# orangeai-research/Generative-Multimodal-Recommendation

Hardware: AMD Instinct MI355X
Metric: train users/sec + full-rank eval users/sec, DiffMM Amazon-baby, 1/2/4/8 MI355X (higher is better)
Workload: dtype fp32; 1 GPU; DiffMM baby-shaped synthetic: 19445 users x 7050 items, 121517 train interactions; step = one DiffMMTrainer epoch (diffusion train + graph rebuild + BPR/contrastive); global_batch=2048, eval_batch=4096, parallelism=dp1

## Files before the change

### generative-multimodal-recommendation_amd/csrc/gemm.hip

```cpp
#include <stdlib.h>

#include <type_traits>

#include "gemm_impl.h"

namespace {
using namespace gmr_gemm;

template <int BM, int BN, int WGM, int WGN, bool AKC, bool BKC, bool VEC, int MF>
__global__ void __launch_bounds__(64 * WGM * WGN) gemm_kernel(int64_t M, int64_t N, int64_t K,
                                                             const float* __restrict__ A, int64_t lda,
                                                             const float* __restrict__ B, int64_t ldb,
                                                             float* __restrict__ C, int64_t ldc, Epi epi, int tiles_n,
                                                             int64_t k_per_split, float* __restrict__ ws) {
  constexpr int NT = 64 * WGM * WGN;
  constexpr int WTM = BM / WGM, WTN = BN / WGN;
  constexpr int TM = WTM / MF, TN = WTN / MF;
  using AccT = typename std::conditional<MF == 32, floatx16, floatx4>::type;
  constexpr int NE = MF == 32 ? 16 : 4;
  using SA = Stage<BM, AKC, VEC, NT>;
  using SB = Stage<BN, BKC, VEC, NT>;
  __shared__ __attribute__((aligned(16))) float smem[2 * (SA::WORDS + SB::WORDS)];
  constexpr int STAGE_WORDS = SA::WORDS + SB::WORDS;

// ... 428 lines not shown
                 int64_t K, const float* A, int64_t lda, const float* B, int64_t ldb, float* C, int64_t ldc,
                 const Epi& epi, int tiles_n, int64_t kps, float* ws, int* counters, bool x6p) {
  if (mf == 6)
    return launch_mf<BM, BN, WGM, WGN, 6>(ta, tb, vec, false, grid, st, M, N, K, A, lda, B, ldb, C, ldc, epi, tiles_n, kps, ws,
                                   counters, x6p);
  else if (mf == 16)
    return launch_mf<BM, BN, WGM, WGN, 16>(ta, tb, vec, false, grid, st, M, N, K, A, lda, B, ldb, C, ldc, epi, tiles_n, kps,
                                    ws, counters, x6p);
  else
    return launch_mf<BM, BN, WGM, WGN, 32>(ta, tb, vec, glds, grid, st, M, N, K, A, lda, B, ldb, C, ldc, epi, tiles_n, kps,
                                    ws, counters, x6p);
}

struct Plan {
  int tile, bm, bn, splits, mf;
  bool glds;
  int64_t tm, tn, kps;
  int xpose;
  bool x6p;
};

int default_mfma() {
  static int mf = [] {
    const char* e = getenv("GMR_GEMM_MFMA");
    return (e && atoi(e) == 16) ? 16 : 32;
  }();
  return mf;
}

bool default_x6() {
  static bool x = [] {
    const char* e = getenv("GMR_GEMM_X6");
    return !(e && atoi(e) == 0);
  }();
  return x;
}

bool default_x6_64() {
  static bool x = [] {
    const char* e = getenv("GMR_GEMM_X6_64");
    return !(e && atoi(e) == 0);
  }();
  return x;
}

bool default_glds() {
  static bool g = [] {
    const char* e = getenv("GMR_GEMM_GLDS");
    return !(e && atoi(e) == 0);
  }();
  return g;
}

int auto_splits(int64_t tm, int64_t tn, int bm, int64_t K) {
  const bool skinny = bm == 64 && (tm == 1 || tn == 1);
  const int64_t min_k = skinny ? 192 : 512;
  const int max_s = skinny ? 64 : 16;
  int s = 1;
  while (tm * tn * s < 512 && K / (s * 2) >= min_k && s < max_s) s *= 2;
  if (bm == 128) {
    const int64_t slots = 512;
    auto waves = [&](int q) { return (double)(tm * tn * q) / (double)slots; };
    auto fill = [&](int q) {
      const int64_t w = tm * tn * q;
      return (double)w / (double)(((w + slots - 1) / slots) * slots);
    };
    while ((waves(s) < 8.0 || fill(s) < 0.9) && K / (s * 2) >= min_k && s < max_s) s *= 2;
  }
  return s;
}

Plan make_plan_core(int ta, int tb, int64_t M, int64_t N, int64_t K, int tile, int split_k, bool allow_x6) {
  int mf = default_mfma();
  if (tile & GMR_GEMM_MFMA16) mf = 16;
  if (tile & GMR_GEMM_MFMA32) mf = 32;
  bool glds = default_glds();
  if (tile & GMR_GEMM_GLDS) glds = true;
  if (tile & GMR_GEMM_REGSTAGE) glds = false;
  const bool x6 = allow_x6 && ((tile & GMR_GEMM_X6) || default_x6()) &&
                  !(tile & (GMR_GEMM_F32 | GMR_GEMM_MFMA16 | GMR_GEMM_MFMA32 | GMR_GEMM_GLDS | GMR_GEMM_REGSTAGE));
  const bool x6_64 = x6 && ((tile & GMR_GEMM_X6) || default_x6_64());
  const bool x6_pipe1 = tile & GMR_GEMM_X6_PIPE1;
  tile &= ~(GMR_GEMM_MFMA16 | GMR_GEMM_MFMA32 | GMR_GEMM_GLDS | GMR_GEMM_REGSTAGE | GMR_GEMM_X6 | GMR_GEMM_F32 |
            GMR_GEMM_X6_PIPE1);
  if (tile == 0) {
    const bool tnm = ta && !tb;
    auto fill = [](int64_t tiles, int64_t slots) { return (double)tiles / (double)(((tiles + slots - 1) / slots) * slots); };
    const bool wide256 = M >= 2048 && N >= 4096 && K >= 256 && K <= 1024 &&
                         fill(((M + 255) / 256) * ((N + 255) / 256), 256) >=
                             0.92 * fill(((M + 127) / 128) * ((N + 127) / 128), 512);
    auto score = [&](int t) {
      const int64_t tm = (M + t - 1) / t, tn = (N + t - 1) / t;
      const int s = auto_splits(tm, tn, t, K);
      double pen = 1.0;
      for (int q = s; q > 1; q >>= 1) pen *= 0.95;
      return fill(tm * tn * s, t == 256 ? 256 : 512) * pen * (t == 256 ? 1.03 : 1.0);
    };
    if (!tnm && M >= 2048 && N >= 1000 && K >= 4096)
      tile = (tb || !glds) && score(256) >= score(128) ? 256 : 128;
    else if (!tnm && wide256) tile = 256;
    else if (!tnm && M * N >= (int64_t)8 << 20 && K >= 512) tile = 128;
    else if (!tnm && M * N >= (int64_t)1 << 20 && K >= 4096) tile = 128;
    else if (!ta && !tb && N <= 64 && M >= 4096 && K >= 2048) tile = 12864;
    else tile = 64;
  }
  if (x6 && tile == 64 && M * N >= ((int64_t)4 << 20) && K >= 256) tile = 128;
  if (x6 && (tile != 64 || x6_64) && tile != 12864 && !ta && tb) {
    mf = 6;
    if (tile == 256) tile = ((M + 127) / 128) * ((N + 127) / 128) >= 768 ? 128 : 256128;
  }
  Plan p;
  p.mf = mf;
  p.glds = glds && mf == 32;
  p.tile = tile;
  p.bm = tile == 256128 ? 256 : tile == 128256 || tile == 12864 ? 128 : tile;
  p.bn = tile == 256128 ? 128 : tile == 128256 ? 256 : tile == 12864 ? 64 : tile;
  p.tm = (M + p.bm - 1) / p.bm;
  p.tn = (N + p.bn - 1) / p.bn;
  int splits = split_k;
  if (splits <= 0 && mf == 6) {
    static const int64_t min_slab_env = [] {
      const char* e = getenv("GMR_X6_MIN_SLAB");
      const int v = e ? atoi(e) : 0;
      return (int64_t)(v >= 64 ? v : 0);
    }();
    const int64_t min_slab = min_slab_env ? min_slab_env : p.bm == 64 ? (x6_ring() && K <= 1024 ? K : 256) : 512;
    const int64_t slots = p.bm == 64 ? 768 : p.bm * p.bn == 128 * 128 ? 512 : 256;
    splits = 1;
    while (p.tm * p.tn * splits * 5 < slots * 4 && K / (splits * 2) >= min_slab && splits < 16) splits *= 2;
  }
  if (splits <= 0) splits = auto_splits(p.tm, p.tn, p.bm, K);
  int64_t kps = (K + splits - 1) / splits;
  kps = (kps + BK - 1) / BK * BK;
  p.splits = (int)((K + kps - 1) / kps);
  p.kps = kps;
  p.xpose = 0;
  p.x6p = mf == 6 && x6_pipe1;
  return p;
}

Plan make_plan(int ta, int tb, int64_t M, int64_t N, int64_t K, int tile, int split_k) {
  if (ta || !tb) {
    Plan q = make_plan_core(0, 1, M, N, K, tile, split_k, true);
    if (q.mf == 6 && q.bm != 64) {
      q.xpose = (ta ? 1 : 0) | (tb ? 0 : 2);
      return q;
    }
    return make_plan_core(ta, tb, M, N, K, tile, split_k, false);
  }
  return make_plan_core(ta, tb, M, N, K, tile, split_k, true);
}

struct WsLayout {
  int64_t slabs, at, bt, total, kp;
};
WsLayout ws_layout(const Plan& p, int64_t M, int64_t N, int64_t K) {
  auto r4 = [](int64_t v) { return (v + 3) / 4 * 4; };
  WsLayout w;
  w.kp = r4(K);
  const bool uses = p.splits > 1 || p.xpose;
  w.slabs = GMR_GEMM_COUNTER_WORDS;
  w.at = uses ? r4(GMR_GEMM_COUNTER_WORDS + (p.splits > 1 ? (int64_t)p.splits * M * N : 0)) : 0;
  w.bt = w.at + ((p.xpose & 1) ? r4(M * w.kp) : 0);
  w.total = w.bt + ((p.xpose & 2) ? r4(N * w.kp) : 0);
  return w;
}

}

extern "C" int32_t gmr_gemm_kernel_kind(int32_t trans_a, int32_t trans_b, int64_t M, int64_t N, int64_t K,
                                        int32_t tile, int32_t split_k, int32_t aligned) {
  if (M <= 0 || N <= 0 || K <= 0) return 0;
  const Plan p = make_plan(trans_a, trans_b, M, N, K, tile, split_k);
  if (p.mf == 6 && !aligned && p.xpose != 3)
    return make_plan_core(trans_a, trans_b, M, N, K, tile, split_k, false).mf;
  return p.mf;
}

extern "C" int64_t gmr_gemm_workspace_floats(int32_t trans_a, int32_t trans_b, int64_t M, int64_t N, int64_t K,
                                             int32_t tile, int32_t split_k) {
  if (M <= 0 || N <= 0 || K <= 0) return 0;
  const Plan p = make_plan(trans_a, trans_b, M, N, K, tile, split_k);
  int64_t need = ws_layout(p, M, N, K).total;
  if (p.mf == 6) {
    const Plan q = make_plan_core(trans_a, trans_b, M, N, K, tile, split_k, false);
    need = std::max(need, ws_layout(q, M, N, K).total);
  }
  return need;
}

extern "C" int gmr_gemm_f32(int32_t trans_a, int32_t trans_b, int64_t M, int64_t N, int64_t K, float alpha,
                            const float* A, int64_t lda, const float* B, int64_t ldb, float beta, float* C,
                            int64_t ldc, int32_t epilogue, const float* bias, const int32_t* bias_row, int64_t ld_bias,
                            const float* aux, int64_t ld_aux, const float* rowvec1, const float* rowvec2, float slope,
                            int32_t tile, int32_t split_k, float* workspace, int64_t workspace_floats, void* stream) {
  GMR_ARG(A && B && C, "null operand");
  GMR_ARG(M > 0 && N > 0 && K > 0, "empty GEMM");
  GMR_ARG(lda >= (trans_a ? M : K) && ldb >= (trans_b ? K : N) && ldc >= N, "leading dimension too small");
  GMR_ARG(epilogue >= GMR_EPI_NONE && epilogue <= GMR_EPI_SCALE_BIAS, "bad epilogue");
  GMR_ARG(epilogue != GMR_EPI_LEAKY_NORM ||
              (N == 64 && aux && rowvec1 && ld_aux >= 64 && ld_aux % 4 == 0 && ldc % 4 == 0 &&
               (((uintptr_t)aux | (uintptr_t)C) & 15) == 0),
          "GMR_EPI_LEAKY_NORM: N = 64, 16-byte aligned C and aux (the normalised rows), rowvec1 (the norms)");
  GMR_ARG(!(epilogue == GMR_EPI_POSTERIOR || epilogue == GMR_EPI_DTANH || epilogue == GMR_EPI_ROWSCALE_AUX ||
            epilogue == GMR_EPI_DRELU) || aux,
          "epilogue needs aux");
  GMR_ARG(epilogue != GMR_EPI_ROWSCALE_AUX || rowvec1, "epilogue needs rowvec1");
  {
    const int t = tile & ~(GMR_GEMM_MFMA16 | GMR_GEMM_MFMA32 | GMR_GEMM_GLDS | GMR_GEMM_REGSTAGE | GMR_GEMM_X6 |
                           GMR_GEMM_F32 | GMR_GEMM_X6_PIPE1);
    GMR_ARG(t == 0 || t == 64 || t == 128 || t == 256 || t == 256128 || t == 128256 || t == 12864,
            "tile must be 0 (auto), 64, 128, 256, 256128, 128256 or 12864 (| GMR_GEMM_MFMA16 / GMR_GEMM_MFMA32)");
  }
  Epi e;
  e.kind = epilogue;
  e.alpha = alpha;
  e.beta = beta;
  e.slope = slope;
  e.bias = bias;
  e.bias_row = bias_row;
  e.ld_bias = ld_bias;
  e.aux = aux;
  e.ld_aux = ld_aux;
  e.rv1 = rowvec1;
  e.rv2 = rowvec2;
  const bool a16 = ((uintptr_t)A % 16 == 0) && lda % 4 == 0, b16 = ((uintptr_t)B % 16 == 0) && ldb % 4 == 0;
  bool vec = a16 && b16;
  Plan pl = make_plan(trans_a, trans_b, M, N, K, tile, split_k);
  if (pl.mf == 6 && !(((pl.xpose & 1) || a16) && ((pl.xpose & 2) || b16)))
    pl = make_plan_core(trans_a, trans_b, M, N, K, tile, split_k, false);
  if ((pl.xpose & 2) && x6_inplace()) pl.xpose &= ~2;
  if (pl.xpose == 1 && !trans_b && x6_inplace() == 2) pl.xpose = 0;
  const WsLayout wl = ws_layout(pl, M, N, K);
  if (pl.xpose) {
    GMR_ARG(workspace && workspace_floats >= wl.total, "needs workspace of gmr_gemm_workspace_floats(...) floats");
    GMR_ARG(((uintptr_t)workspace & 15) == 0, "workspace must be 16-byte aligned");
    if (pl.xpose & 1) {
      x6_transpose(A, lda, K, M, workspace + wl.at, wl.kp, (hipStream_t)stream);
      GMR_LAUNCHED();
      A = workspace + wl.at;
      lda = wl.kp;
    }
    if (pl.xpose & 2) {
      x6_transpose(B, ldb, K, N, workspace + wl.bt, wl.kp, (hipStream_t)stream);
      GMR_LAUNCHED();
      B = workspace + wl.bt;
      ldb = wl.kp;
    }
    if (pl.xpose & 1) trans_a = 0;
    if (pl.xpose & 2) trans_b = 1;
    vec = (pl.xpose & 1 ? true : a16) && (pl.xpose & 2 ? true : b16);
  }
  tile = pl.tile;
  const int64_t tm = pl.tm, tn = pl.tn, kps = pl.kps;
  const int splits = pl.splits;
  GMR_ARG(tm * tn < (1ll << 31), "too many tiles");
  float* ws = nullptr;
  int* counters = nullptr;
  if (splits > 1) {
    GMR_ARG(workspace && workspace_floats >= GMR_GEMM_COUNTER_WORDS + (int64_t)splits * M * N,
            "split-K needs workspace of gmr_gemm_workspace_floats(...) floats");
    ws = workspace + GMR_GEMM_COUNTER_WORDS;
    if (pl.glds && vec && tm * tn <= GMR_GEMM_COUNTER_WORDS && inkernel_fixup() && epilogue != GMR_EPI_LEAKY_NORM)
      counters = reinterpret_cast<int*>(workspace);
  }
  GMR_ARG(epilogue != GMR_EPI_LEAKY_NORM || splits > 1, "GMR_EPI_LEAKY_NORM needs a split-K plan");
  hipStream_t st = (hipStream_t)stream;
  dim3 grid((unsigned)(tm * tn), 1, (unsigned)splits);
  const int tnp = (int)tn | (tile_group(tn) << 20);
  int lrc = 0;
  switch (tile) {
    case 256:
      lrc = launch_tile<256, 256, 4, 4>(pl.mf, pl.glds, trans_a, trans_b, vec, grid, st, M, N, K, A, lda, B, ldb, C, ldc, e, tnp, kps, ws, counters, pl.x6p);
      break;
    case 256128:
      lrc = launch_tile<256, 128, 4, 2>(pl.mf, pl.glds, trans_a, trans_b, vec, grid, st, M, N, K, A, lda, B, ldb, C, ldc, e, tnp, kps, ws, counters, pl.x6p);
      break;
    case 128256:
      lrc = launch_tile<128, 256, 2, 4>(pl.mf, pl.glds, trans_a, trans_b, vec, grid, st, M, N, K, A, lda, B, ldb, C, ldc, e, tnp, kps, ws, counters, pl.x6p);
      break;
    case 12864:
      lrc = launch_tile<128, 64, 2, 2>(pl.mf, pl.glds, trans_a, trans_b, vec, grid, st, M, N, K, A, lda, B, ldb, C, ldc, e, tnp, kps, ws, counters, pl.x6p);
      break;
    case 128:
      lrc = launch_tile<128, 128, 2, 2>(pl.mf, pl.glds, trans_a, trans_b, vec, grid, st, M, N, K, A, lda, B, ldb, C, ldc, e, tnp, kps, ws, counters, pl.x6p);
      break;
    default:
      lrc = launch_tile<64, 64, 2, 2>(pl.mf, pl.glds, trans_a, trans_b, vec, grid, st, M, N, K, A, lda, B, ldb, C, ldc, e, tnp, kps, ws, counters, pl.x6p);
  }
  GMR_ARG(lrc == 0, "no split-bf16 kernel for this tile and operand layout");
  GMR_LAUNCHED();
  if (ws && !counters && epilogue == GMR_EPI_LEAKY_NORM) {
    hipLaunchKernelGGL(splitk_reduce_leaky_norm_kernel, dim3(gmr::grid_for(M * 16, 256)), dim3(256), 0, st, M, splits,
                       ws, C, ldc, e, const_cast<float*>(aux), ld_aux, const_cast<float*>(rowvec1));
    GMR_LAUNCHED();
  } else if (ws && !counters) {
    hipLaunchKernelGGL(splitk_reduce_kernel, dim3(gmr::grid_for(M * N, 256)), dim3(256), 0, st, M, N, splits, ws, C,
                       ldc, e);
    GMR_LAUNCHED();
  }
  return GMR_OK;
}
```

### generative-multimodal-recommendation_amd/csrc/gemm_x6.hip

```cpp
#include <stdlib.h>

#include <type_traits>

#include "gemm_impl.h"
#include "x6_split.h"

namespace {
using namespace gmr_gemm;

typedef __bf16 bf16x8 __attribute__((ext_vector_type(8)));
typedef __bf16 bf16x4 __attribute__((ext_vector_type(4)));

__device__ __forceinline__ int x6_swz(int r) { return (r >> 2) & 3; }

__device__ __forceinline__ void split3(float x, __bf16& h, __bf16& m, __bf16& l) {
  h = (__bf16)__builtin_amdgcn_fmed3f(x, -0x1.fep127f, 0x1.fep127f);
  const float r1 = x - (float)h;
  m = (__bf16)r1;
  l = (__bf16)(r1 - (float)m);
}

template <int N, typename V>
__device__ __forceinline__ void split3n(const float* v, V& h, V& m, V& l) {
  typedef unsigned U __attribute__((ext_vector_type(N / 2)));
  U hh, mm, ll;
#pragma unroll
  for (int e = 0; e < N / 2; ++e) {
    unsigned a, b, c;
    gmr_x6::split_pair(v[2 * e], v[2 * e + 1], a, b, c);
    hh[e] = a, mm[e] = b, ll[e] = c;
  }
  h = __builtin_bit_cast(V, hh);
  m = __builtin_bit_cast(V, mm);
  l = __builtin_bit_cast(V, ll);
}

template <int R, bool KC, int NT, int N4>
__device__ __forceinline__ void x6_store(const float4 (&r)[N4], __bf16* s) {
  constexpr int PL = R * BK;
  const int t = threadIdx.x;
#pragma unroll
  for (int i = 0; i < N4; ++i) {
    const int idx = t + NT * i;
    const float v[4] = {r[i].x, r[i].y, r[i].z, r[i].w};
    if (KC) {
      const int rr = idx / (BK / 4), k4 = (idx % (BK / 4)) * 4;
      bf16x4 h, m, l;
      split3n<4>(v, h, m, l);
      const int off = rr * BK + (((k4 >> 3) ^ x6_swz(rr)) << 3) + (k4 & 7);
      *reinterpret_cast<bf16x4*>(s + off) = h;
      *reinterpret_cast<bf16x4*>(s + PL + off) = m;
      *reinterpret_cast<bf16x4*>(s + 2 * PL + off) = l;
    } else {
      const int kk = idx / (R / 4), m4 = (idx % (R / 4)) * 4;
#pragma unroll
      for (int e = 0; e < 4; ++e) {
        const int rr = m4 + e;
        const int off = rr * BK + (((kk >> 3) ^ x6_swz(rr)) << 3) + (kk & 7);
        __bf16 a, b, c;
        split3(v[e], a, b, c);
        s[off] = a;
        s[PL + off] = b;
        s[2 * PL + off] = c;
      }
    }
  }
}

template <int R, int NT>
struct KcTile {
  static constexpr int N4 = R * BK / 4 / NT;
  static_assert(N4 * NT * 4 == R * BK, "tile rows x BK must split evenly over the block");
  int off[N4];
  float4 r[N4];

  __device__ __forceinline__ void init(int64_t r0, int64_t nrows, int64_t ld) {
#pragma unroll
    for (int i = 0; i < N4; ++i) {
      const int idx = threadIdx.x + NT * i;
      const int rr = idx / (BK / 4), k4 = (idx % (BK / 4)) * 4;
      const int64_t row = min(r0 + rr, nrows - 1) - r0;
      off[i] = (int)(row * ld) + k4;
    }
  }
  __device__ __forceinline__ void load(const float* __restrict__ base) {
#pragma unroll
    for (int i = 0; i < N4; ++i) r[i] = *reinterpret_cast<const float4*>(base + off[i]);
  }
  __device__ __forceinline__ void load_tail(const float* __restrict__ base, int kleft) {
#pragma unroll
    for (int i = 0; i < N4; ++i) {
      const int k4 = ((threadIdx.x + NT * i) % (BK / 4)) * 4;
      float4 v = make_float4(0.f, 0.f, 0.f, 0.f);
      if (k4 < kleft) {
        v = *reinterpret_cast<const float4*>(base + off[i]);
        if (k4 + 1 >= kleft) v.y = 0.f;
        if (k4 + 2 >= kleft) v.z = 0.f;
        if (k4 + 3 >= kleft) v.w = 0.f;
      }
      r[i] = v;
    }
  }
};

template <int R, int NT>
struct MnTile {
  static constexpr int E = R * BK / NT;
  static_assert(E % 8 == 0 && NT % R == 0, "whole 8-k chunks of one row per thread");
  int off;
  int rr;
  int kt;
  int64_t ld;
  float v[E];

  __device__ __forceinline__ void init(int64_t r0, int64_t nrows, int64_t ld_) {
    ld = ld_;
    rr = threadIdx.x % R;
    kt = (threadIdx.x / R) * E;
    off = (int)(kt * ld + (min(r0 + rr, nrows - 1) - r0));
  }
  __device__ __forceinline__ void load(const float* __restrict__ base, int kleft) {
#pragma unroll
    for (int e = 0; e < E; ++e) v[e] = (kleft == BK || kt + e < kleft) ? base[off + e * ld] : 0.f;
  }
  __device__ __forceinline__ void store(__bf16* s) const {
    constexpr int PL = R * BK;
#pragma unroll
    for (int c = 0; c < E / 8; ++c) {
      bf16x8 h, m, l;
      split3n<8>(v + 8 * c, h, m, l);
      const int o = rr * BK + ((((kt >> 3) + c) ^ x6_swz(rr)) << 3);
      *reinterpret_cast<bf16x8*>(s + o) = h;
      *reinterpret_cast<bf16x8*>(s + PL + o) = m;
      *reinterpret_cast<bf16x8*>(s + 2 * PL + o) = l;
    }
  }
};

template <int R, int NT, int N4>
__device__ __forceinline__ void kc_fetch(float4 (&d)[N4], const KcTile<R, NT>& tl, const float* __restrict__ base,
                                         bool full, int kleft) {
  if (full) {
#pragma unroll
    for (int i = 0; i < N4; ++i) d[i] = *reinterpret_cast<const float4*>(base + tl.off[i]);
  } else {
#pragma unroll
    for (int i = 0; i < N4; ++i) {
      const int k4 = ((threadIdx.x + NT * i) % (BK / 4)) * 4;
      float4 v = make_float4(0.f, 0.f, 0.f, 0.f);
      if (k4 < kleft) {
        v = *reinterpret_cast<const float4*>(base + tl.off[i]);
        if (k4 + 1 >= kleft) v.y = 0.f;
        if (k4 + 2 >= kleft) v.z = 0.f;
        if (k4 + 3 >= kleft) v.w = 0.f;
      }
      d[i] = v;
    }
  }
}

template <int BM, int BN, int WGM, int WGN, int NBUF, int OCC, int PIPE, bool AKC = true, bool BKC = true>
__global__ void __launch_bounds__(64 * WGM * WGN, OCC) gemm_x6_kernel(int64_t M, int64_t N, int64_t K,
                                                                const float* __restrict__ A, int64_t lda,
                                                                const float* __restrict__ B, int64_t ldb,
                                                                float* __restrict__ C, int64_t ldc, Epi epi,
                                                                int tiles_n, int64_t k_per_split,
                                                                float* __restrict__ ws) {
  constexpr int NT = 64 * WGM * WGN;
  constexpr int WTM = BM / WGM, WTN = BN / WGN;
  constexpr int TM = WTM / 32, TN = WTN / 32;
  constexpr int APL = BM * BK, BPL = BN * BK;
  constexpr int STAGE = 3 * (APL + BPL);
  __shared__ __attribute__((aligned(16))) __bf16 smem[NBUF * STAGE];

  const int nwg = gridDim.x;
  const int b = blockIdx.x;
  const int xcd = b & 7, q = nwg >> 3, r = nwg & 7;
  const int tile = (xcd < r ? xcd * (q + 1) : r * (q + 1) + (xcd - r) * q) + (b >> 3);
  int tmi, tni;
  tile_mn(tile, tiles_n, (int)((M + BM - 1) / BM), tmi, tni);
  const int64_t m0 = (int64_t)tmi * BM;
  const int64_t n0 = (int64_t)tni * BN;
  const int64_t kbeg = (int64_t)blockIdx.z * k_per_split;
  const int64_t kend = min(K, kbeg + k_per_split);

  const int lane = threadIdx.x & 63;
  const int w = threadIdx.x >> 6;
  const int wm = w / WGN, wn = w % WGN;
  const int h = lane >> 5, l32 = lane & 31;

  floatx16 acc[TM][TN], sml[TM][TN];
#pragma unroll
  for (int i = 0; i < TM; ++i)
#pragma unroll
    for (int j = 0; j < TN; ++j)
#pragma unroll
      for (int e = 0; e < 16; ++e) acc[i][j][e] = sml[i][j][e] = 0.f;

  auto mstep = [&](const __bf16* a_s, int s, auto&& gap) {
    const __bf16* b_s = a_s + 3 * APL;
    bf16x8 fb[3][TN];
#pragma unroll
    for (int j = 0; j < TN; ++j) {
      const int row = wn * WTN + j * 32 + l32;
      const int off = row * BK + (((2 * s + h) ^ x6_swz(row)) << 3);
#pragma unroll
      for (int p = 0; p < 3; ++p) fb[p][j] = *reinterpret_cast<const bf16x8*>(b_s + p * BPL + off);
    }
    bf16x8 fa_[TM][3];
    auto read_a = [&](int i) {
      const int row = wm * WTM + i * 32 + l32;
      const int off = row * BK + (((2 * s + h) ^ x6_swz(row)) << 3);
#pragma unroll
      for (int p = 0; p < 3; ++p) fa_[i][p] = *reinterpret_cast<const bf16x8*>(a_s + p * APL + off);
    };
    if constexpr (PIPE == 1) {
#pragma unroll
      for (int i = 0; i < TM; ++i) read_a(i);
      __builtin_amdgcn_sched_barrier(0);
    }
#pragma unroll
    for (int i = 0; i < TM; ++i) {
      if constexpr (PIPE != 1) read_a(i);
      const bf16x8(&fa)[3] = fa_[i];
#pragma unroll
      for (int j = 0; j < TN; ++j) {
        const int g = 6 * (i * TN + j);
        sml[i][j] = __builtin_amdgcn_mfma_f32_32x32x16_bf16(fa[1], fb[1][j], sml[i][j], 0, 0, 0);
        gap(g);
        sml[i][j] = __builtin_amdgcn_mfma_f32_32x32x16_bf16(fa[0], fb[2][j], sml[i][j], 0, 0, 0);
        gap(g + 1);
        sml[i][j] = __builtin_amdgcn_mfma_f32_32x32x16_bf16(fa[2], fb[0][j], sml[i][j], 0, 0, 0);
        gap(g + 2);
        sml[i][j] = __builtin_amdgcn_mfma_f32_32x32x16_bf16(fa[0], fb[1][j], sml[i][j], 0, 0, 0);
        gap(g + 3);
        sml[i][j] = __builtin_amdgcn_mfma_f32_32x32x16_bf16(fa[1], fb[0][j], sml[i][j], 0, 0, 0);
        gap(g + 4);
        acc[i][j] = __builtin_amdgcn_mfma_f32_32x32x16_bf16(fa[0], fb[0][j], acc[i][j], 0, 0, 0);
        gap(g + 5);
      }
    }
  };

  auto nogap = [](int) {};
  static_assert((AKC && BKC) || PIPE == 0, "m- / n-contiguous operands: the PIPE 0 loop only");
  std::conditional_t<AKC, KcTile<BM, NT>, MnTile<BM, NT>> ra;
  std::conditional_t<BKC, KcTile<BN, NT>, MnTile<BN, NT>> rb;
  ra.init(m0, M, lda);
  rb.init(n0, N, ldb);
  const float* a0 = AKC ? A + m0 * lda : A + m0;
  const float* b0 = BKC ? B + n0 * ldb : B + n0;
  const int nk = kend > kbeg ? (int)((kend - kbeg + BK - 1) / BK) : 0;
  const int kl = (int)(kend - kbeg - (int64_t)(nk - 1) * BK);
  auto fetch = [&](int t) {
    const int64_t k0 = kbeg + (int64_t)t * BK;
    if constexpr (AKC && BKC) {
      if (t + 1 < nk || kl == BK) {
        ra.load(a0 + k0);
        rb.load(b0 + k0);
      } else {
        ra.load_tail(a0 + k0, kl);
        rb.load_tail(b0 + k0, kl);
      }
    } else {
      const int kleft = t + 1 < nk ? BK : kl;
      if constexpr (AKC) {
        if (kleft == BK) ra.load(a0 + k0);
        else ra.load_tail(a0 + k0, kleft);
      } else {
        ra.load(a0 + k0 * lda, kleft);
      }
      rb.load(b0 + k0 * ldb, kleft);
    }
  };
  auto store = [&](__bf16* s) {
    if constexpr (AKC) x6_store<BM, true, NT>(ra.r, s);
    else ra.store(s);
    if constexpr (BKC) x6_store<BN, true, NT>(rb.r, s + 3 * APL);
    else rb.store(s + 3 * APL);
  };
  if constexpr (PIPE == 2) {
    constexpr int PF = 4;
    constexpr int NA = KcTile<BM, NT>::N4, NB = KcTile<BN, NT>::N4;
    float4 qa[PF][NA], qb[PF][NB];
    auto fetch_slot = [&](float4 (&da)[NA], float4 (&db)[NB], int t) {
      if (t < nk) {
        const int64_t k0 = kbeg + (int64_t)t * BK;
        const bool full = t + 1 < nk || kl == BK;
        kc_fetch<BM, NT, NA>(da, ra, a0 + k0, full, kl);
        kc_fetch<BN, NT, NB>(db, rb, b0 + k0, full, kl);
      }
    };
#pragma unroll
    for (int q = 0; q < PF; ++q) fetch_slot(qa[q], qb[q], q);
    for (int t0 = 0; t0 < nk; t0 += PF) {
#pragma unroll
      for (int q = 0; q < PF; ++q) {
        const int t = t0 + q;
        if (t < nk) {
          __bf16* buf = smem + (t & 1) * STAGE;
          x6_store<BM, true, NT>(qa[q], buf);
          x6_store<BN, true, NT>(qb[q], buf + 3 * APL);
          __syncthreads();
          fetch_slot(qa[q], qb[q], t + PF);
          mstep(buf, 0, nogap);
          mstep(buf, 1, nogap);
        }
      }
    }
    __syncthreads();
  } else if constexpr (PIPE == 0) {
  int cur = 0;
  if (nk > 0) {
    fetch(0);
    store(smem);
  }
  __syncthreads();
  for (int t = 0; t < nk; ++t) {
    const bool more = t + 1 < nk;
    if (more) fetch(t + 1);
    const __bf16* a_s = smem + cur * STAGE;
    mstep(a_s, 0, nogap);
    mstep(a_s, 1, nogap);
    if constexpr (NBUF == 2) {
      if (more) store(smem + (cur ^ 1) * STAGE);
      __syncthreads();
      cur ^= 1;
    } else {
      __syncthreads();
      if (more) store(smem);
      __syncthreads();
    }
  }
  } else {
    static_assert(NBUF == 2, "the pipelined loop double-buffers LDS");
    constexpr int NA = KcTile<BM, NT>::N4, NB = KcTile<BN, NT>::N4, NF = NA + NB;
    constexpr int NM = 6 * TM * TN;
    constexpr int NPC = 6 * NF;
    constexpr int PPG = (NPC + 2 * NM - 1) / (2 * NM);
    float4 qa[NA], qb[NB];
    auto fetch_next = [&](int t) {
      fetch(min(t, nk - 1));
    };
    if (nk > 0) {
      fetch(0);
      x6_store<BM, true, NT>(ra.r, smem);
      x6_store<BN, true, NT>(rb.r, smem + 3 * APL);
      fetch_next(1);
    }
    __syncthreads();
    for (int t = 0; t < nk; ++t) {
#pragma unroll
      for (int i = 0; i < NA; ++i) qa[i] = ra.r[i];
#pragma unroll
      for (int i = 0; i < NB; ++i) qb[i] = rb.r[i];
// ... 24 lines not shown
      auto gap0 = [&](int g) {
#pragma unroll
        for (int c = g * PPG; c < (g + 1) * PPG; ++c)
          if (c < NPC) piece(c);
        __builtin_amdgcn_sched_barrier(0);
      };
      auto gap1 = [&](int g) { gap0(NM + g); };
      mstep(a_s, 0, gap0);
      mstep(a_s, 1, gap1);
      __syncthreads();
    }
  }

#pragma unroll
  for (int i = 0; i < TM; ++i)
#pragma unroll
    for (int j = 0; j < TN; ++j) acc[i][j] += sml[i][j];

  if (!ws && epi_reads_x(epi))
    gemm_epilogue_lds<BM, BN, WGM, WGN, NBUF * 3 * (BM + BN) * BK / 2>(acc, reinterpret_cast<float*>(smem), M, N, C,
                                                                     ldc, epi, m0, n0, ws);
  else
    gemm_epilogue<BM, BN, WGM, WGN, 32>(acc, M, N, C, ldc, epi, m0, n0, ws);
}

__global__ void __launch_bounds__(256) x6_transpose_kernel(const float* __restrict__ src, int64_t ld_src,
                                                           int64_t rows, int64_t cols, float* __restrict__ dst,
                                                           int64_t ld_dst, int64_t tiles_c) {
  __shared__ float t[64][65];
  const int64_t tr = blockIdx.x / tiles_c, tc = blockIdx.x % tiles_c;
  const int64_t r0 = tr * 64, c0 = tc * 64;
  const int x = threadIdx.x & 63, y = threadIdx.x >> 6;
#pragma unroll
  for (int i = 0; i < 16; ++i) {
    const int64_t r = r0 + y + 4 * i, c = c0 + x;
    t[y + 4 * i][x] = (r < rows && c < cols) ? src[r * ld_src + c] : 0.f;
  }
  __syncthreads();
#pragma unroll
  for (int i = 0; i < 16; ++i) {
    const int64_t c = c0 + y + 4 * i, r = r0 + x;
    if (c < cols && r < rows) dst[c * ld_dst + r] = t[x][y + 4 * i];
  }
}

}

namespace gmr_gemm {

void x6_transpose(const float* src, int64_t ld_src, int64_t rows, int64_t cols, float* dst, int64_t ld_dst,
                  hipStream_t st) {
  const int64_t tr = (rows + 63) / 64, tc = (cols + 63) / 64;
  hipLaunchKernelGGL(x6_transpose_kernel, dim3((unsigned)(tr * tc)), dim3(256), 0, st, src, ld_src, rows, cols, dst,
                     ld_dst, tc);
}

static int x6_pipe() {
  static const int v = [] {
    const char* e = getenv("GMR_GEMM_X6_PIPE");
    return e ? atoi(e) : -1;
  }();
  return v;
}

int x6_ring() {
  static const int v = [] {
    const char* e = getenv("GMR_X6_RING");
    return e ? atoi(e) : 1;
  }();
  return v;
}

static int x6_nb128() {
  static const int v = [] {
    const char* e = getenv("GMR_GEMM_X6_NB128");
    return e ? atoi(e) : 0;
  }();
  return v;
}

int x6_inplace() {
  static const int v = [] {
    const char* e = getenv("GMR_X6_INPLACE");
    return e ? atoi(e) : 0;
  }();
  return v;
}

int x6_launch(int bm, int bn, dim3 grid, hipStream_t st, int64_t M, int64_t N, int64_t K, const float* A, int64_t lda,
              const float* B, int64_t ldb, float* C, int64_t ldc, const Epi& epi, int tiles_n, int64_t kps, float* ws,
              bool akc, bool bkc, bool pipe) {
  if (x6_pipe() == 0 || x6_pipe() == 1) pipe = x6_pipe() == 1;
  if (x6_pipe() == 2) pipe = pipe || bm * bn == 256 * 128;
#define GMR_X6(BM_, BN_, WGM_, WGN_, NBUF_, OCC_)                                                                \
  {                                                                                                                \
    if (!akc || !bkc) {                                                                                            \
      if (akc)                                                                                                     \
        hipLaunchKernelGGL((gemm_x6_kernel<BM_, BN_, WGM_, WGN_, NBUF_, OCC_, 0, true, false>), grid,              \
                           dim3(64 * WGM_ * WGN_), 0, st, M, N, K, A, lda, B, ldb, C, ldc, epi, tiles_n, kps, ws); \
      else if (!bkc)                                                                                               \
        hipLaunchKernelGGL((gemm_x6_kernel<BM_, BN_, WGM_, WGN_, NBUF_, OCC_, 0, false, false>), grid,             \
                           dim3(64 * WGM_ * WGN_), 0, st, M, N, K, A, lda, B, ldb, C, ldc, epi, tiles_n, kps, ws); \
      else                                                                                                         \
        return -1;                                                                                                 \
      return 0;                                                                                                    \
    }                                                                                                              \
    if (NBUF_ == 2 && pipe)                                                                                        \
      hipLaunchKernelGGL((gemm_x6_kernel<BM_, BN_, WGM_, WGN_, NBUF_, OCC_, NBUF_ - 1>), grid, dim3(64 * WGM_ * WGN_), \
                         0, st, M, N, K, A, lda, B, ldb, C, ldc, epi, tiles_n, kps, ws);                           \
    else                                                                                                           \
      hipLaunchKernelGGL((gemm_x6_kernel<BM_, BN_, WGM_, WGN_, NBUF_, OCC_, 0>), grid, dim3(64 * WGM_ * WGN_), 0,   \
                         st, M, N, K, A, lda, B, ldb, C, ldc, epi, tiles_n, kps, ws);                              \
    return 0;                                                                                                      \
  }
  if (bm == 64 && bn == 64 && (!akc || !bkc)) return -1;
  if (bm == 64 && bn == 64 && x6_ring()) {
    hipLaunchKernelGGL((gemm_x6_kernel<64, 64, 2, 2, 2, 3, 2>), grid, dim3(256), 0, st, M, N, K, A, lda, B, ldb, C,
                       ldc, epi, tiles_n, kps, ws);
    return 0;
  }
  if (bm == 64 && bn == 64) GMR_X6(64, 64, 2, 2, 2, 3)
  if (bm == 256 && bn == 128) GMR_X6(256, 128, 4, 2, 2, 1)
  if (bm == 128 && bn == 256) GMR_X6(128, 256, 2, 4, 2, 1)
  if (bm == 128 && bn == 128) {
    const int nb = x6_nb128();
    if (nb == 2 || (pipe && akc && bkc && nb == 0)) GMR_X6(128, 128, 2, 2, 2, 1)
    if (nb == 3) GMR_X6(128, 128, 2, 2, 1, 3)
    GMR_X6(128, 128, 2, 2, 1, 2)
  }
#undef GMR_X6
  return -1;
}

}
```

### generative-multimodal-recommendation_amd/gmr/kernels.py

```python
import ctypes
import os

import torch

from . import _lib

EPI_NONE, EPI_BIAS, EPI_BIAS_TANH, EPI_LEAKY, EPI_POSTERIOR, EPI_DTANH, EPI_ROWSCALE_AUX, EPI_BIAS_RELU, EPI_DRELU = range(9)
EPI_LEAKY_NORM = 9
EPI_SCALE_BIAS = 10

_ws = {}

_probe = None
_probe_every = 1
_probe_count = 0


def probe_begin(tags, every=1):
    global _probe, _probe_every, _probe_count
    _probe = {t: [] for t in tags}
    _probe_every, _probe_count = max(1, int(every)), 0


def probe_end():
# ... 80 lines not shown

    def __del__(self):
        try:
            self.close()
        except Exception:
            pass


Streams.SERIAL = os.environ.get("GMR_SERIAL", "0") == "1"


class _OnSide:
    __slots__ = ("st", "i", "prev", "ctx")

    def __init__(self, st, i):
        self.st, self.i = st, i

    def __enter__(self):
        st, i = self.st, self.i
        if Streams.SERIAL:
            self.prev = None
            return None
        if _cur_device is not None and _cur_device() != st._dev:
            raise RuntimeError(f"Streams built on device {st._dev} used while device {_cur_device()} is current")
        _lib.call("gmr_stream_fork", stream(), st._raw[i], st._ev[2 * i])
        pb = Streams.PERTURB
        if pb is not None and pb[1] == i:
            _lib.call("gmr_delay", int(pb[2]), st._raw[i] if pb[0] == "side" else stream())
        if _get_stream is None or _set_stream is None:
            self.prev = None
            self.ctx = torch.cuda.stream(st.side[i])
            self.ctx.__enter__()
            return st.side[i]
        self.ctx = None
        self.prev = _get_stream(st._dev)
        sid, dev, dt = st._ids[i]
        _set_stream(stream_id=sid, device_index=dev, device_type=dt)
        return st.side[i]

    def __exit__(self, *a):
        if self.prev is None:
            if not Streams.SERIAL and self.ctx is not None:
                self.ctx.__exit__(*a)
            return False
        sid, dev, dt = self.prev
        _set_stream(stream_id=sid, device_index=dev, device_type=dt)
        return False


def ptr(t):
    if t is None:
        return None
    if not t.is_cuda:
        raise ValueError("gmr kernels take device tensors only (no CPU fallback)")
    return ctypes.c_void_p(t.data_ptr())


def _ld(t):
    if t.dim() == 1:
        return t.shape[0]
    if t.stride(-1) != 1:
        raise ValueError("inner dimension must be contiguous")
    return t.stride(0)


def workspace(nfloats, device, tag="gemm"):
    key = (tag, device, _raw_stream(_cur_device()) if _raw_stream is not None and _cur_device is not None
           else torch.cuda.current_stream().cuda_stream)
    w = _ws.get(key)
    if w is None or w.numel() < nfloats:
        w = torch.zeros(max(nfloats, 1 << 20), dtype=torch.float32, device=device)
        _ws[key] = w
    return w


def zero_(t):
    if not t.is_contiguous():
        raise ValueError("zero_ needs a contiguous tensor")
    _lib.call("gmr_zero", ptr(t), t.numel() * t.element_size(), stream())
    return t


_gemm_kinds = {}
GEMM_TILE_FLAGS = 0


def _gemm_tag(A, B, trans_a, trans_b, M, N, K, tile, split_k):
    aligned = int(A.data_ptr() % 16 == 0 and B.data_ptr() % 16 == 0 and _ld(A) % 4 == 0 and _ld(B) % 4 == 0)
    key = (int(trans_a), int(trans_b), M, N, K, tile, split_k, aligned)
    kind = _gemm_kinds.get(key)
    if kind is None:
        kind = _gemm_kinds[key] = int(_lib.load().gmr_gemm_kernel_kind(*key))
    return "gemm_x6" if kind == 6 else "gemm"


_gemm_plans = {}


def _gemm_plan(A, B, C, trans_a, trans_b, tile, split_k):
    M, N = C.shape
    K = A.shape[0] if trans_a else A.shape[1]
    if (A.shape[1] if trans_a else A.shape[0]) != M:
        raise ValueError(f"A shape {tuple(A.shape)} does not give M={M}")
    if (B.shape[1] if trans_b else B.shape[0]) != K or (B.shape[0] if trans_b else B.shape[1]) != N:
        raise ValueError(f"B shape {tuple(B.shape)} does not match K={K}, N={N}")
    for t in (A, B, C):
        if t.dtype != torch.float32:
            raise TypeError("gemm is fp32")
        if not t.is_cuda:
            raise ValueError("gmr kernels take device tensors only (no CPU fallback)")
    tile |= GEMM_TILE_FLAGS
    need = int(_lib.load().gmr_gemm_workspace_floats(int(trans_a), int(trans_b), M, N, K, tile, split_k))
    return M, N, K, tile, need, _ld(A), _ld(B), _ld(C)


def gemm(A, B, C, trans_a=False, trans_b=False, alpha=1.0, beta=0.0, epi=EPI_NONE, bias=None, bias_row=None,
         ld_bias=0, aux=None, rv1=None, rv2=None, slope=0.0, tile=0, split_k=0):
    key = (A.shape, A.stride(), B.shape, B.stride(), C.shape, C.stride(), A.dtype, B.dtype, C.dtype, A.device,
           trans_a, trans_b, tile, split_k, GEMM_TILE_FLAGS)
    pl = _gemm_plans.get(key)
    if pl is None:
        pl = _gemm_plans[key] = _gemm_plan(A, B, C, trans_a, trans_b, tile, split_k)
    M, N, K, tile, need, lda, ldb, ldc = pl
    ws = workspace(need, C.device) if need > 0 else None
    args = (int(trans_a), int(trans_b), M, N, K, float(alpha), A.data_ptr(), lda, B.data_ptr(), ldb, float(beta),
            C.data_ptr(), ldc, epi, ptr(bias), ptr(bias_row), ld_bias, ptr(aux), _ld(aux) if aux is not None else 0,
            ptr(rv1), ptr(rv2), float(slope), tile, split_k, ws.data_ptr() if ws is not None else None,
            ws.numel() if ws is not None else 0, stream())
    if _probe is None:
        _lib.call("gmr_gemm_f32", *args)
    else:
        with _Probe(_gemm_tag(A, B, trans_a, trans_b, M, N, K, tile, split_k), (M, N, K, int(trans_a), int(trans_b), epi)):
            _lib.call("gmr_gemm_f32", *args)
    return C


class Planes:

    def __init__(self, rows, cols, device):
        self.rows, self.cols = int(rows), int(cols)
        self.ld = (self.cols + 31) // 32 * 32
        self.t = torch.zeros((3, self.rows, self.ld), dtype=torch.int16, device=device)
        self.ps = self.rows * self.ld

    def ptr(self):
        return ctypes.c_void_p(self.t.data_ptr())

    def load(self, src):
        if src.shape[0] > self.rows or src.shape[1] != self.cols or src.dtype != torch.float32 or src.stride(1) != 1:
            raise ValueError("split3: src must be an fp32 (<= rows) x cols matrix with unit column stride")
        _lib.call("gmr_split3_planes", src.shape[0], self.cols, ptr(src), src.stride(0), self.ptr(), self.ld, self.ps,
                  stream())
        return self

    def to_float(self):
        p = self.t[:, :, :self.cols].to(torch.int32) << 16
        f = p.view(torch.float32) if p.is_contiguous() else p.contiguous().view(torch.float32)
        return (f[0] + f[1]) + f[2]


SPMM_CLASSES = os.environ.get("GMR_SPMM_CLASSES", "0") == "1"
SPMM_NO_SPLIT_ROWS = 1
SPMM_HUB_FIXUP = 2
SPMM_LANE_PLAN = 1 << 16
SPMM_PACKED = 1 << 17
SPMM_SEG_NNZ = SPMM_LANE_PLAN | 32
# ... 451 lines not shown
```

### include/gmr.h

```cpp
#ifndef GMR_H_
#define GMR_H_

#include <stdint.h>

#ifdef __cplusplus
extern "C" {
#endif

#define GMR_ABI_VERSION 2
#define GMR_OK 0
#define GMR_ERR_ARG (-1000)

#define GMR_EPI_NONE 0
#define GMR_EPI_BIAS 1
#define GMR_EPI_BIAS_TANH 2
#define GMR_EPI_LEAKY 3
#define GMR_EPI_POSTERIOR 4
#define GMR_EPI_DTANH 5
#define GMR_EPI_ROWSCALE_AUX 6
#define GMR_EPI_BIAS_RELU 7
#define GMR_GEMM_COUNTER_WORDS 16384
#define GMR_GEMM_GLDS (1 << 22)
#define GMR_GEMM_REGSTAGE (1 << 23)
#define GMR_GEMM_MFMA16 (1 << 24)
#define GMR_GEMM_MFMA32 (1 << 25)
#define GMR_GEMM_X6 (1 << 26)
#define GMR_GEMM_F32 (1 << 27)
#define GMR_GEMM_X6_PIPE1 (1 << 28)
#define GMR_EPI_DRELU 8
#define GMR_EPI_LEAKY_NORM 9
#define GMR_EPI_SCALE_BIAS 10

const char* gmr_last_error_string(void);
int gmr_version(void);
int gmr_device_name(char* buf , int32_t len);
int gmr_zero(void* ptr, int64_t bytes, void* stream);
int gmr_event_create(void** ev );
int gmr_event_destroy(void* ev);
int gmr_stream_fork(void* from, void* to, void* ev);
int gmr_delay(int32_t us, void* stream);

#define GMR_SPMM_NO_SPLIT_ROWS 1
#define GMR_SPMM_HUB_FIXUP 2
#define GMR_SPMM_LANE_PLAN (1 << 16)
#define GMR_SPMM_PACKED (1 << 17)
#define GMR_SPMM_CHUNK_PLAN (1 << 18)
int64_t gmr_spmm_plan_words(int64_t n_rows, int64_t nnz, int32_t seg_nnz);
int64_t gmr_spmm_partial_rows(int64_t n_rows, int64_t nnz, int32_t seg_nnz);
int gmr_spmm_plan_build_split(const int32_t* rowptr, int64_t n_rows, int64_t nnz, int32_t seg_nnz,
                              int64_t class_split, int32_t* plan, void* stream);
int gmr_spmm_plan_build(const int32_t* rowptr, int64_t n_rows, int64_t nnz, int32_t seg_nnz, int32_t* plan,
                        void* stream);
int gmr_spmm_plan_pack(const int32_t* rowptr, const int32_t* col, const float* val, int64_t n_rows, int64_t nnz,
                       int32_t seg_nnz, int32_t* plan, void* stream);
int gmr_spmm_panel_f32(const int32_t* col, const float* val, int64_t n_rows, int64_t nnz, const int32_t* plan,
                       int32_t seg_nnz, int32_t n_blocks, const float* x_panel, int64_t panel_rows, float alpha,
                       float beta, float* y, int64_t ldy, float* partial, int32_t flags, void* stream);
int gmr_spmm_multi_f32(const int32_t* col, const float* val, int64_t n_rows, int64_t nnz, const int32_t* plan,
                       int32_t seg_nnz, int32_t n_blocks, const float* const* x_lo, const int64_t* ld_lo,
                       const float* const* x_hi, const int64_t* ld_hi, int64_t split, float alpha, float beta,
                       float* const* y_blocks, const int64_t* ld_y, float* partial, int32_t flags, void* stream);
typedef struct gmr_spmm_job {
  const int32_t* col;
  const float* val;
  const int32_t* plan;
  float* partial;
  int64_t n_rows, nnz;
  int32_t seg_nnz, n_blocks, flags, reserved;
  const float* x_lo[4];
  int64_t ld_lo[4];
  const float* x_hi[4];
  int64_t ld_hi[4];
  int64_t split;
  float alpha, beta;
  float* y[4];
  int64_t ld_y[4];
} gmr_spmm_job;
int gmr_spmm_jobs_f32(int32_t n_jobs, const gmr_spmm_job* jobs, void* stream);
int gmr_spmm_plan_info(const int32_t* plan, int32_t* host_hdr, void* stream);

#define GMR_SIDE_CLASSES (1 << 24)
int64_t gmr_spmm_side_plan_words(const int32_t* rowptr_host, int64_t n_rows, int64_t split, int32_t T);
int gmr_spmm_side_plan_build(const int32_t* rowptr_host, int64_t n_rows, int64_t split, int32_t T, int32_t* plan_host,
                             int64_t words);
int64_t gmr_spmm_side_scratch_floats(const int32_t* plan_host);
int gmr_spmm_side_pack(const int32_t* rowptr, const int32_t* col, const float* val, int64_t n_rows, int64_t nnz,
                       int64_t packed_off, int32_t* plan, void* stream);
int gmr_spmm_side_pack_classes(const int32_t* rowptr, const int32_t* col, const float* val, const int32_t* plan_host,
                               int32_t* plan, void* stream);
int gmr_spmm_side_tune(int32_t wpx, int32_t eb);
int gmr_spmm_side_f32(const int32_t* plan, int32_t n_blocks, const float* const* x_lo, const int64_t* ld_lo,
                      const float* const* x_hi, const int64_t* ld_hi, int64_t split, float alpha, float beta,
                      float* const* y_blocks, const int64_t* ld_y, float* scratch, int32_t wpx, void* stream);
int gmr_spmm_side2_f32(const int32_t* plan, int32_t n_blocks, const float* const* x_lo, const int64_t* ld_lo,
                       const float* const* x_hi, const int64_t* ld_hi, int64_t split, float alpha, float beta,
                       const float* const* z_blocks, const int64_t* ld_z, float* const* y_blocks, const int64_t* ld_y,
                       int32_t only_side, float* scratch, int32_t wpx, void* stream);
int gmr_spmm_side_jobs_f32(int32_t njobs, const int32_t* const* plans, float* const* scratch, int32_t n_blocks,
                           const float* const* x_lo, const int64_t* ld_lo, const float* const* x_hi,
                           const int64_t* ld_hi, const int64_t* split, float alpha, float beta, float* const* y,
                           const int64_t* ld_y, int32_t wpx, void* stream);

int gmr_spmm_csr_f32(const int32_t* rowptr, const int32_t* col, const float* val, int64_t n_rows, int64_t nnz,
                     const int32_t* plan, int32_t seg_nnz, float* partial, int32_t n_blocks,
                     const float* const* x_lo, const int64_t* ld_lo, const float* const* x_hi, const int64_t* ld_hi,
                     int64_t split, float alpha, float beta, float* y, int64_t ldy, int32_t flags, void* stream);

int gmr_score_f16(int64_t E, int64_t I, int64_t d, const float* A, int64_t lda, const float* B, int64_t ldb,
                  float* C, int64_t ldc, void* stream);

int64_t gmr_bipartite_nnz(int64_t n_users, int64_t n_items, int64_t n_user_items, int32_t self_loops);
// ... 511 lines not shown
```

Baseline: 311,100 users/s.

## Read m/n-contiguous x6 GEMM operands in place via LDS transpose reads

The x6 split-bf16 GEMM now loads m- or n-contiguous operands directly with float4 loads into a k-major LDS layout, then builds MFMA fragments with ds_read_tr16_b64 transpose reads. The old per-element strided loader is replaced. By default, the separate transpose-to-workspace kernel is skipped when alignment and leading dimensions allow, with a new X6_COPY flag to force the old copy path. This removes extra transpose launches and workspace traffic, at the cost of a more complex swizzled LDS path and possible bank conflicts or slower fragment reads.

New measurement: 317,300 users/s, median of 6. +2.0%, better.

```diff
diff --git a/generative-multimodal-recommendation_amd/csrc/gemm.hip b/generative-multimodal-recommendation_amd/csrc/gemm.hip
--- a/generative-multimodal-recommendation_amd/csrc/gemm.hip
+++ b/generative-multimodal-recommendation_amd/csrc/gemm.hip
@@ -534,7 +534,7 @@
   const bool x6_64 = x6 && ((tile & GMR_GEMM_X6) || default_x6_64());
   const bool x6_pipe1 = tile & GMR_GEMM_X6_PIPE1;
   tile &= ~(GMR_GEMM_MFMA16 | GMR_GEMM_MFMA32 | GMR_GEMM_GLDS | GMR_GEMM_REGSTAGE | GMR_GEMM_X6 | GMR_GEMM_F32 |
-            GMR_GEMM_X6_PIPE1);
+            GMR_GEMM_X6_PIPE1 | GMR_GEMM_X6_COPY);
   if (tile == 0) {
     const bool tnm = ta && !tb;
     auto fill = [](int64_t tiles, int64_t slots) { return (double)tiles / (double)(((tiles + slots - 1) / slots) * slots); };
@@ -660,7 +660,7 @@
   GMR_ARG(epilogue != GMR_EPI_ROWSCALE_AUX || rowvec1, "epilogue needs rowvec1");
   {
     const int t = tile & ~(GMR_GEMM_MFMA16 | GMR_GEMM_MFMA32 | GMR_GEMM_GLDS | GMR_GEMM_REGSTAGE | GMR_GEMM_X6 |
-                           GMR_GEMM_F32 | GMR_GEMM_X6_PIPE1);
+                           GMR_GEMM_F32 | GMR_GEMM_X6_PIPE1 | GMR_GEMM_X6_COPY);
     GMR_ARG(t == 0 || t == 64 || t == 128 || t == 256 || t == 256128 || t == 128256 || t == 12864,
             "tile must be 0 (auto), 64, 128, 256, 256128, 128256 or 12864 (| GMR_GEMM_MFMA16 / GMR_GEMM_MFMA32)");
   }
@@ -681,8 +681,11 @@
   Plan pl = make_plan(trans_a, trans_b, M, N, K, tile, split_k);
   if (pl.mf == 6 && !(((pl.xpose & 1) || a16) && ((pl.xpose & 2) || b16)))
     pl = make_plan_core(trans_a, trans_b, M, N, K, tile, split_k, false);
-  if ((pl.xpose & 2) && x6_inplace()) pl.xpose &= ~2;
-  if (pl.xpose == 1 && !trans_b && x6_inplace() == 2) pl.xpose = 0;
+  if (pl.mf == 6 && pl.xpose && !trans_b && !(tile & GMR_GEMM_X6_COPY) && x6_inplace() != 0) {
+    auto r4 = [](int64_t v) { return (v + 3) / 4 * 4; };
+    if (b16 && ldb >= r4(N)) pl.xpose &= ~2;
+    if ((pl.xpose & 1) && x6_inplace() != 1 && a16 && lda >= r4(M)) pl.xpose &= ~1;
+  }
   const WsLayout wl = ws_layout(pl, M, N, K);
   if (pl.xpose) {
     GMR_ARG(workspace && workspace_floats >= wl.total, "needs workspace of gmr_gemm_workspace_floats(...) floats");
diff --git a/generative-multimodal-recommendation_amd/csrc/gemm_x6.hip b/generative-multimodal-recommendation_amd/csrc/gemm_x6.hip
--- a/generative-multimodal-recommendation_amd/csrc/gemm_x6.hip
+++ b/generative-multimodal-recommendation_amd/csrc/gemm_x6.hip
@@ -104,38 +104,66 @@
 };
 
 template <int R, int NT>
-struct MnTile {
-  static constexpr int E = R * BK / NT;
-  static_assert(E % 8 == 0 && NT % R == 0, "whole 8-k chunks of one row per thread");
-  int off;
-  int rr;
-  int kt;
-  int64_t ld;
-  float v[E];
-
-  __device__ __forceinline__ void init(int64_t r0, int64_t nrows, int64_t ld_) {
-    ld = ld_;
-    rr = threadIdx.x % R;
-    kt = (threadIdx.x / R) * E;
-    off = (int)(kt * ld + (min(r0 + rr, nrows - 1) - r0));
+struct TrTile {
+  static constexpr int N4 = R * BK / 4 / NT;
+  static constexpr int GR = R / 4;
+  static_assert(N4 * NT * 4 == R * BK && NT % (4 * GR) == 0, "whole k rows per pass, k & 3 fixed per thread");
+  static_assert(R % 128 == 0, "the swizzle moves a unit by up to 24 within its k row, a 32-row block by up to 3");
+  int off[N4];
+  float4 r[N4];
+
+  __device__ __forceinline__ void init(int64_t r0, int64_t nrows, int64_t ld) {
+    const int last = (int)(((nrows - 1) & ~(int64_t)3) - r0);
+#pragma unroll
+    for (int i = 0; i < N4; ++i) {
+      const int idx = threadIdx.x + NT * i;
+      const int kk = idx / GR, m4 = (idx % GR) * 4;
+      off[i] = (int)(kk * ld) + min(m4, last);
+    }
   }
   __device__ __forceinline__ void load(const float* __restrict__ base, int kleft) {
-#pragma unroll
-    for (int e = 0; e < E; ++e) v[e] = (kleft == BK || kt + e < kleft) ? base[off + e * ld] : 0.f;
+    if (kleft == BK) {
+#pragma unroll
+      for (int i = 0; i < N4; ++i) r[i] = *reinterpret_cast<const float4*>(base + off[i]);
+    } else {
+#pragma unroll
+      for (int i = 0; i < N4; ++i) {
+        const int kk = (threadIdx.x + NT * i) / GR;
+        r[i] = kk < kleft ? *reinterpret_cast<const float4*>(base + off[i]) : make_float4(0.f, 0.f, 0.f, 0.f);
+      }
+    }
   }
   __device__ __forceinline__ void store(__bf16* s) const {
     constexpr int PL = R * BK;
 #pragma unroll
-    for (int c = 0; c < E / 8; ++c) {
-      bf16x8 h, m, l;
-      split3n<8>(v + 8 * c, h, m, l);
-      const int o = rr * BK + ((((kt >> 3) + c) ^ x6_swz(rr)) << 3);
-      *reinterpret_cast<bf16x8*>(s + o) = h;
-      *reinterpret_cast<bf16x8*>(s + PL + o) = m;
-      *reinterpret_cast<bf16x8*>(s + 2 * PL + o) = l;
+    for (int i = 0; i < N4; ++i) {
+      const int idx = threadIdx.x + NT * i;
+      const int kk = idx / GR, u = idx % GR;
+      const float v[4] = {r[i].x, r[i].y, r[i].z, r[i].w};
+      bf16x4 h, m, l;
+      split3n<4>(v, h, m, l);
+      const int o = kk * R + ((u ^ ((kk & 3) << 3)) << 2);
+      *reinterpret_cast<bf16x4*>(s + o) = h;
+      *reinterpret_cast<bf16x4*>(s + PL + o) = m;
+      *reinterpret_cast<bf16x4*>(s + 2 * PL + o) = l;
     }
   }
 };
+
+template <int R>
+__device__ __forceinline__ int x6_tr_lane_off(int J) {
+  const int lane = threadIdx.x & 63;
+  const int q = (lane & 15) >> 2, p = lane & 3, gs = (lane >> 4) & 1, h = lane >> 5;
+  return (8 * h + q) * R + ((((J ^ q) << 3) + 4 * gs + p) << 2);
+}
+
+template <int R>
+__device__ __forceinline__ bf16x8 x6_tr_frag(const __bf16* pl, int o, int s) {
+  typedef __attribute__((address_space(3))) bf16x4* lds4;
+  const bf16x4 a = __builtin_amdgcn_ds_read_tr16_b64_v4bf16((lds4)(pl + o + 16 * s * R));
+  const bf16x4 b = __builtin_amdgcn_ds_read_tr16_b64_v4bf16((lds4)(pl + o + (16 * s + 4) * R));
+  return __builtin_shufflevector(a, b, 0, 1, 2, 3, 4, 5, 6, 7);
+}
 
 template <int R, int NT, int N4>
 __device__ __forceinline__ void kc_fetch(float4 (&d)[N4], const KcTile<R, NT>& tl, const float* __restrict__ base,
@@ -197,22 +225,38 @@
 #pragma unroll
       for (int e = 0; e < 16; ++e) acc[i][j][e] = sml[i][j][e] = 0.f;
 
+  [[maybe_unused]] int tra[TM], trb[TN];
+#pragma unroll
+  for (int i = 0; i < TM; ++i) tra[i] = AKC ? 0 : x6_tr_lane_off<BM>(wm * (WTM / 32) + i);
+#pragma unroll
+  for (int j = 0; j < TN; ++j) trb[j] = BKC ? 0 : x6_tr_lane_off<BN>(wn * (WTN / 32) + j);
+
   auto mstep = [&](const __bf16* a_s, int s, auto&& gap) {
     const __bf16* b_s = a_s + 3 * APL;
     bf16x8 fb[3][TN];
 #pragma unroll
     for (int j = 0; j < TN; ++j) {
-      const int row = wn * WTN + j * 32 + l32;
-      const int off = row * BK + (((2 * s + h) ^ x6_swz(row)) << 3);
-#pragma unroll
-      for (int p = 0; p < 3; ++p) fb[p][j] = *reinterpret_cast<const bf16x8*>(b_s + p * BPL + off);
+      if constexpr (BKC) {
+        const int row = wn * WTN + j * 32 + l32;
+        const int off = row * BK + (((2 * s + h) ^ x6_swz(row)) << 3);
+#pragma unroll
+        for (int p = 0; p < 3; ++p) fb[p][j] = *reinterpret_cast<const bf16x8*>(b_s + p * BPL + off);
+      } else {
+#pragma unroll
+        for (int p = 0; p < 3; ++p) fb[p][j] = x6_tr_frag<BN>(b_s + p * BPL, trb[j], s);
+      }
     }
     bf16x8 fa_[TM][3];
     auto read_a = [&](int i) {
-      const int row = wm * WTM + i * 32 + l32;
-      const int off = row * BK + (((2 * s + h) ^ x6_swz(row)) << 3);
-#pragma unroll
-      for (int p = 0; p < 3; ++p) fa_[i][p] = *reinterpret_cast<const bf16x8*>(a_s + p * APL + off);
+      if constexpr (AKC) {
+        const int row = wm * WTM + i * 32 + l32;
+        const int off = row * BK + (((2 * s + h) ^ x6_swz(row)) << 3);
+#pragma unroll
+        for (int p = 0; p < 3; ++p) fa_[i][p] = *reinterpret_cast<const bf16x8*>(a_s + p * APL + off);
+      } else {
+#pragma unroll
+        for (int p = 0; p < 3; ++p) fa_[i][p] = x6_tr_frag<BM>(a_s + p * APL, tra[i], s);
+      }
     };
     if constexpr (PIPE == 1) {
 #pragma unroll
@@ -244,8 +288,8 @@
 
   auto nogap = [](int) {};
   static_assert((AKC && BKC) || PIPE == 0, "m- / n-contiguous operands: the PIPE 0 loop only");
-  std::conditional_t<AKC, KcTile<BM, NT>, MnTile<BM, NT>> ra;
-  std::conditional_t<BKC, KcTile<BN, NT>, MnTile<BN, NT>> rb;
+  std::conditional_t<AKC, KcTile<BM, NT>, TrTile<BM, NT>> ra;
+  std::conditional_t<BKC, KcTile<BN, NT>, TrTile<BN, NT>> rb;
   ra.init(m0, M, lda);
   rb.init(n0, N, ldb);
   const float* a0 = AKC ? A + m0 * lda : A + m0;
@@ -270,7 +314,12 @@
       } else {
         ra.load(a0 + k0 * lda, kleft);
       }
-      rb.load(b0 + k0 * ldb, kleft);
+      if constexpr (BKC) {
+        if (kleft == BK) rb.load(b0 + k0);
+        else rb.load_tail(b0 + k0, kleft);
+      } else {
+        rb.load(b0 + k0 * ldb, kleft);
+      }
     }
   };
   auto store = [&](__bf16* s) {
@@ -461,9 +510,30 @@
 int x6_inplace() {
   static const int v = [] {
     const char* e = getenv("GMR_X6_INPLACE");
-    return e ? atoi(e) : 0;
+    return e ? atoi(e) : -1;
   }();
   return v;
+}
+
+template <int BM, int BN, int WGM, int WGN, int NBUF, int OCC>
+static int x6_launch_tr(bool akc, bool bkc, dim3 grid, hipStream_t st, int64_t M, int64_t N, int64_t K, const float* A,
+                        int64_t lda, const float* B, int64_t ldb, float* C, int64_t ldc, const Epi& epi, int tiles_n,
+                        int64_t kps, float* ws) {
+  if constexpr (BM % 128 == 0 && BN % 128 == 0) {
+    const dim3 blk(64 * WGM * WGN);
+    if (akc)
+      hipLaunchKernelGGL((gemm_x6_kernel<BM, BN, WGM, WGN, NBUF, OCC, 0, true, false>), grid, blk, 0, st, M, N, K, A, lda,
+                         B, ldb, C, ldc, epi, tiles_n, kps, ws);
+    else if (!bkc)
+      hipLaunchKernelGGL((gemm_x6_kernel<BM, BN, WGM, WGN, NBUF, OCC, 0, false, false>), grid, blk, 0, st, M, N, K, A, lda,
+                         B, ldb, C, ldc, epi, tiles_n, kps, ws);
+    else
+      hipLaunchKernelGGL((gemm_x6_kernel<BM, BN, WGM, WGN, NBUF, OCC, 0, false, true>), grid, blk, 0, st, M, N, K, A, lda,
+                         B, ldb, C, ldc, epi, tiles_n, kps, ws);
+    return 0;
+  } else {
+    return -1;
+  }
 }
 
 int x6_launch(int bm, int bn, dim3 grid, hipStream_t st, int64_t M, int64_t N, int64_t K, const float* A, int64_t lda,
@@ -473,17 +543,9 @@
   if (x6_pipe() == 2) pipe = pipe || bm * bn == 256 * 128;
 #define GMR_X6(BM_, BN_, WGM_, WGN_, NBUF_, OCC_)                                                                \
   {                                                                                                                \
-    if (!akc || !bkc) {                                                                                            \
-      if (akc)                                                                                                     \
-        hipLaunchKernelGGL((gemm_x6_kernel<BM_, BN_, WGM_, WGN_, NBUF_, OCC_, 0, true, false>), grid,              \
-                           dim3(64 * WGM_ * WGN_), 0, st, M, N, K, A, lda, B, ldb, C, ldc, epi, tiles_n, kps, ws); \
-      else if (!bkc)                                                                                               \
-        hipLaunchKernelGGL((gemm_x6_kernel<BM_, BN_, WGM_, WGN_, NBUF_, OCC_, 0, false, false>), grid,             \
-                           dim3(64 * WGM_ * WGN_), 0, st, M, N, K, A, lda, B, ldb, C, ldc, epi, tiles_n, kps, ws); \
-      else                                                                                                         \
-        return -1;                                                                                                 \
-      return 0;                                                                                                    \
-    }                                                                                                              \
+    if (!akc || !bkc)                                                                                              \
+      return x6_launch_tr<BM_, BN_, WGM_, WGN_, NBUF_, OCC_>(akc, bkc, grid, st, M, N, K, A, lda, B, ldb, C, ldc, epi, \
+                                                             tiles_n, kps, ws);                                   \
     if (NBUF_ == 2 && pipe)                                                                                        \
       hipLaunchKernelGGL((gemm_x6_kernel<BM_, BN_, WGM_, WGN_, NBUF_, OCC_, NBUF_ - 1>), grid, dim3(64 * WGM_ * WGN_), \
                          0, st, M, N, K, A, lda, B, ldb, C, ldc, epi, tiles_n, kps, ws);                           \
diff --git a/generative-multimodal-recommendation_amd/gmr/kernels.py b/generative-multimodal-recommendation_amd/gmr/kernels.py
--- a/generative-multimodal-recommendation_amd/gmr/kernels.py
+++ b/generative-multimodal-recommendation_amd/gmr/kernels.py
@@ -186,6 +186,7 @@
 
 
 _gemm_kinds = {}
+GEMM_X6_COPY = 1 << 29
 GEMM_TILE_FLAGS = 0
 
 
diff --git a/include/gmr.h b/include/gmr.h
--- a/include/gmr.h
+++ b/include/gmr.h
@@ -27,6 +27,7 @@
 #define GMR_GEMM_X6 (1 << 26)
 #define GMR_GEMM_F32 (1 << 27)
 #define GMR_GEMM_X6_PIPE1 (1 << 28)
+#define GMR_GEMM_X6_COPY (1 << 29)
 #define GMR_EPI_DRELU 8
 #define GMR_EPI_LEAKY_NORM 9
 #define GMR_EPI_SCALE_BIAS 10
```
